# yahoojapan/srgd

Hardware: AMD Instinct MI355X
Metric: HR tiles/sec (256->1024 x4, 50 steps, CFG=1.0) (higher is better)
Workload: dtype bf16; 1 GPU; BASELINE configs[1]: one 256x256 LR tile x4 SR per step, 50 DDPM steps, class_cond_scale=1.0, dim-128 U-Net, bf16, device Philox noise; 5 steps (HR tiles) advance in lock-step so their U-Net tiles share launches; images_in_lockstep=5, step_lanes=1, tiles_per_unet_launch=125, parallelism=image-sharded x1

## Files before the change

srgd_amd/csrc/conv1x1_bf16.hip:

```cpp
#include "conv1x1_epilogue.hpp"

namespace srgd {
namespace {

constexpr int BM1 = 256, BN1 = 128, KC1 = 32, NT1 = 512;
constexpr int A1_BYTES = BM1 * KC1 * 2;
constexpr int B1_BYTES = BN1 * KC1 * 2;
constexpr int STAGE1 = A1_BYTES + B1_BYTES;
constexpr int RING1 = 3;
constexpr int LDS1_BYTES = RING1 * STAGE1;
static_assert(LDS1_BYTES >= EPI_LDS_BYTES && BM1 == EPI_BM && BN1 == EPI_BN && NT1 == EPI_NT, "conv1x1_epilogue.hpp tile shape");

typedef __attribute__((address_space(3))) void* lds_ptr1;
__device__ __forceinline__ void dma16_1(__amdgpu_buffer_rsrc_t rsrc, char* lds_wave_base, int voffset, int soffset) {
  __builtin_amdgcn_raw_ptr_buffer_load_lds(rsrc, (lds_ptr1)lds_wave_base, 16, voffset, soffset, 0, 0);
}
#define WAIT_VM1(N) asm volatile("s_waitcnt vmcnt(" #N ")" ::: "memory")
#define BARRIER1()                       \
  do {                                   \
    __builtin_amdgcn_s_barrier();        \
    __builtin_amdgcn_sched_barrier(0);   \
  } while (0)

struct Conv1Args {
  const bf16* in0; const bf16* in1; int C0, C1;
  int B, Hin, Win;
  int Hout, Wout;
  int KH, KW, stride;
  int ps0, ps1;
  const bf16* w;
  const float* bias;
  int Cout;
  bf16* out;
  const bf16* aux;
  const float* gn_a; const float* gn_b;
  unsigned char* oq; unsigned char* os;
  float* eps4; const float* fin_w; const float* fin_b;
};

__device__ __forceinline__ int row_swz1(int row) { return (row >> 1) & 3; }

template <int EPI>
__global__ __launch_bounds__(NT1, 4) void conv1x1_bf16_kernel(Conv1Args p) {
  extern __shared__ __attribute__((aligned(16))) char smem[];
  const int tid = threadIdx.x;
  const int lane = tid & 63;
  const int wave = __builtin_amdgcn_readfirstlane(tid >> 6);
  const int wm = wave >> 1, wn = wave & 1;
  const int r16 = lane & 15, q16 = lane >> 4;

  const int n_tiles = p.Cout / BN1;
  const int HWo = p.Hout * p.Wout;
  int wg = blockIdx.x;
  {
    const int nwg = gridDim.x, q = nwg >> 3, rem = nwg & 7, x = wg & 7, k = wg >> 3;
    wg = (x < rem ? x * (q + 1) : rem * (q + 1) + (x - rem) * q) + k;
  }
  const int nt = wg % n_tiles;
  const int mt = wg / n_tiles;
  const long m0 = (long)mt * BM1;
  const int b = (int)(m0 / HWo);
  const int p0 = (int)(m0 - (long)b * HWo);
  const int Cin = p.C0 + p.C1;
  const int CC = Cin / KC1;
  const int S = p.KH * p.KW * CC;

#define K_A1_DECL(J)                                                      \
  int a_b0##J, a_b1##J;                                                      \
  {                                                                          \
    const int g = (wave + 8 * J) * 64 + lane;                                \
    const int P = g >> 2;                                                    \
    const int op = p0 + P;                                                   \
    const int oy = op / p.Wout, ox = op - oy * p.Wout;                       \
    const int pix = oy * p.stride * p.Win + ox * p.stride;                   \
    const int sub = (g & 3) ^ row_swz1(P);                                   \
    a_b0##J = (pix * p.ps0 + sub * 8) * 2;                                   \
    a_b1##J = (pix * p.ps1 + sub * 8) * 2;                                   \
  }
  K_A1_DECL(0) K_A1_DECL(1)
#undef K_A1_DECL
  const size_t img0 = (size_t)p.Hin * p.Win * p.ps0, img1 = (size_t)p.Hin * p.Win * p.ps1;
  const __amdgpu_buffer_rsrc_t rs0 =
      __builtin_amdgcn_make_buffer_rsrc((void*)(p.in0 + (size_t)b * img0), 0, (int)(img0 * 2), 0x00020000);
  const __amdgpu_buffer_rsrc_t rs1 = __builtin_amdgcn_make_buffer_rsrc(
      (void*)(p.in1 ? p.in1 + (size_t)b * img1 : p.in0), 0, p.in1 ? (int)(img1 * 2) : 0, 0x00020000);
  const size_t w_tile_stride = (size_t)n_tiles * B1_BYTES;
  const __amdgpu_buffer_rsrc_t rsw = __builtin_amdgcn_make_buffer_rsrc(
      (void*)((const char*)p.w + (size_t)nt * B1_BYTES), 0, (int)((size_t)(S - 1) * w_tile_stride + B1_BYTES), 0x00020000);

  int i_ty = 0, i_tx = 0, i_cc = 0, i_slot = 0, i_w = 0;
  const int tid16 = tid * 16;
  auto issue = [&]() __attribute__((always_inline)) {
    const int c = i_cc * KC1;
    const bool first = c < p.C0;
    const int soff = first ? ((i_ty * p.Win + i_tx) * p.ps0 + c) * 2 : ((i_ty * p.Win + i_tx) * p.ps1 + c - p.C0) * 2;
    char* st = smem + i_slot * STAGE1;
    const int vo0 = first ? a_b00 : a_b10, vo1 = first ? a_b01 : a_b11;
    if (first) {
      dma16_1(rs0, st + wave * 1024, vo0, soff);
      dma16_1(rs0, st + (wave + 8) * 1024, vo1, soff);
    } else {
      dma16_1(rs1, st + wave * 1024, vo0, soff);
      dma16_1(rs1, st + (wave + 8) * 1024, vo1, soff);
    }
    dma16_1(rsw, st + A1_BYTES + wave * 1024, tid16, i_w);
    i_w += (int)w_tile_stride;
    i_slot = i_slot == RING1 - 1 ? 0 : i_slot + 1;
    if (++i_cc == CC) {
      i_cc = 0;
      if (++i_tx == p.KW) { i_tx = 0; ++i_ty; }
    }
  };

  f32x4 c00 = 0, c01 = 0, c02 = 0, c03 = 0, c10 = 0, c11 = 0, c12 = 0, c13 = 0,
        c20 = 0, c21 = 0, c22 = 0, c23 = 0, c30 = 0, c31 = 0, c32 = 0, c33 = 0;
  auto a_addr = [&](int i) {
    const int P = wm * 64 + i * 16 + r16;
    return P * 64 + ((q16 ^ row_swz1(P)) << 4);
  };
  auto b_addr = [&](int j) {
    const int n = wn * 64 + j * 16 + r16;
    return A1_BYTES + n * 64 + ((q16 ^ row_swz1(n)) << 4);
  };
  const int aa0 = a_addr(0), aa1 = a_addr(1), aa2 = a_addr(2), aa3 = a_addr(3);
  const int ba0 = b_addr(0), ba1 = b_addr(1), ba2 = b_addr(2), ba3 = b_addr(3);
  int c_slot = 0;
  auto compute = [&]() __attribute__((always_inline)) {
    const char* st = smem + c_slot * STAGE1;
    c_slot = c_slot == RING1 - 1 ? 0 : c_slot + 1;
    const bf16x8 a0 = *reinterpret_cast<const bf16x8*>(st + aa0);
    const bf16x8 a1 = *reinterpret_cast<const bf16x8*>(st + aa1);
    const bf16x8 a2 = *reinterpret_cast<const bf16x8*>(st + aa2);
    const bf16x8 a3 = *reinterpret_cast<const bf16x8*>(st + aa3);
    const bf16x8 b0 = *reinterpret_cast<const bf16x8*>(st + ba0);
    const bf16x8 b1 = *reinterpret_cast<const bf16x8*>(st + ba1);
    const bf16x8 b2 = *reinterpret_cast<const bf16x8*>(st + ba2);
    const bf16x8 b3 = *reinterpret_cast<const bf16x8*>(st + ba3);
#define MM(C_, A_, B_) C_ = __builtin_amdgcn_mfma_f32_16x16x32_bf16(A_, B_, C_, 0, 0, 0)
    MM(c00, a0, b0); MM(c01, a0, b1); MM(c02, a0, b2); MM(c03, a0, b3);
    MM(c10, a1, b0); MM(c11, a1, b1); MM(c12, a1, b2); MM(c13, a1, b3);
    MM(c20, a2, b0); MM(c21, a2, b1); MM(c22, a2, b2); MM(c23, a2, b3);
    MM(c30, a3, b0); MM(c31, a3, b1); MM(c32, a3, b2); MM(c33, a3, b3);
#undef MM
  };

  issue();
  if (S > 1) issue();
  if (S > 1) WAIT_VM1(3); else WAIT_VM1(0);
  BARRIER1();
  for (int s = 0; s < S; ++s) {
    if (s + 2 < S) issue();
    compute();
    if (s + 2 < S) WAIT_VM1(3); else WAIT_VM1(0);
    BARRIER1();
  }

  conv1x1_epilogue<EPI, BM1>(p, smem, tid, nt, m0, b, p0, c00, c01, c02, c03, c10, c11, c12, c13, c20, c21, c22, c23, c30, c31, c32, c33);
}

}

bool conv1x1_bf16_eligible(const ConvArgs& a) {
  if (a.pad != 0 || a.stride < 1 || a.KH < 1 || a.KW < 1) return false;
  if ((a.Hout - 1) * a.stride + a.KH > a.Hin || (a.Wout - 1) * a.stride + a.KW > a.Win) return false;
  if (a.ps0 % 8 || (a.C1 && (a.ps1 % 8 || a.ps1 < a.C1))) return false;
  if (a.ps0 != a.C0 && (a.C1 || (long)(a.Win - (a.Wout - 1) * a.stride - a.KW) * a.ps0 + a.ps0 < a.C0)) return false;
  if (a.C1 && (a.KH != 1 || a.KW != 1)) return false;
  if (a.C0 % KC1 || a.C1 % KC1 || a.Cout % BN1 || a.Cout != a.CoutPad) return false;
  if (((long)a.Hout * a.Wout) % BM1) return false;
  if (a.gn_partial) return false;
  if (a.mode == CONV_PIXEL_SHUFFLE_SILU && ((a.Cout / 4) % BN1 || a.residual || a.gn_res_src)) return false;
  if (a.mode != CONV_PLAIN && a.mode != CONV_PIXEL_SHUFFLE_SILU) return false;
  if (a.residual && a.gn_res_src) return false;
  if (a.eps4 && (!a.gn_res_src || a.Cout != BN1 || !a.fin_w || !a.fin_b || a.out_q)) return false;
  if ((size_t)a.Hin * a.Win * (size_t)std::max(a.ps0, a.ps1) * 2 >= (1ull << 31)) return false;
  if ((size_t)a.KH * a.KW * ((a.C0 + a.C1) / KC1) * (a.Cout / BN1) * B1_BYTES >= (1ull << 31)) return false;
  return true;
}

void pack_conv1x1_bf16(const float* src_tap_o_i, int taps, int Cin, int Cout, std::vector<unsigned short>& out,
                       unsigned short (*to_bf16)(float)) {
  const int CC = Cin / KC1, NTL = Cout / BN1;
  out.assign((size_t)taps * CC * NTL * BN1 * KC1, 0);
  for (int tap = 0; tap < taps; ++tap)
    for (int cc = 0; cc < CC; ++cc)
      for (int nt = 0; nt < NTL; ++nt) {
        unsigned short* tile = out.data() + ((size_t)(tap * CC + cc) * NTL + nt) * BN1 * KC1;
        for (int n = 0; n < BN1; ++n)
          for (int c = 0; c < 4; ++c) {
            const int cs = c ^ ((n >> 1) & 3);
            for (int e = 0; e < 8; ++e) {
              const int ci = cc * KC1 + c * 8 + e, o = nt * BN1 + n;
              tile[n * KC1 + cs * 8 + e] = to_bf16(src_tap_o_i[((size_t)tap * Cout + o) * Cin + ci]);
            }
          }
      }
}

int conv1x1_bf16(const ConvArgs& a, const void* packed_w, hipStream_t st) {
  if (!conv1x1_bf16_eligible(a)) SRGD_FAIL("conv1x1_bf16: shape not eligible");
  Conv1Args p;
  p.in0 = (const bf16*)a.in0; p.in1 = (const bf16*)a.in1; p.C0 = a.C0; p.C1 = a.C1;
  p.B = a.B; p.Hin = a.Hin; p.Win = a.Win; p.Hout = a.Hout; p.Wout = a.Wout;
  p.KH = a.KH; p.KW = a.KW; p.stride = a.stride; p.ps0 = a.ps0; p.ps1 = a.C1 ? a.ps1 : 0;
  p.w = (const bf16*)packed_w; p.bias = a.bias; p.Cout = a.Cout; p.out = (bf16*)a.out;
  p.aux = a.gn_res_src ? (const bf16*)a.gn_res_src : (const bf16*)a.residual;
  p.gn_a = a.gn_res_a; p.gn_b = a.gn_res_b;
  p.oq = (unsigned char*)a.out_q; p.os = (unsigned char*)a.out_s;
  p.eps4 = a.eps4; p.fin_w = a.fin_w; p.fin_b = a.fin_b;
  if ((p.oq != nullptr) != (p.os != nullptr)) SRGD_FAIL("conv1x1_bf16: MX-fp8 twin needs both the element and the scale buffer");
  const long m_tiles = (long)a.B * a.Hout * a.Wout / BM1;
  const long grid = m_tiles * (a.Cout / BN1);
  if (grid <= 0 || grid > 0x7fffffffL) SRGD_FAIL("conv1x1_bf16: bad grid");
  static bool attr_set[64] = {};
  if (DeviceSetup once(attr_set); once.need) {
#define K_SET1(E_)                                                                                   \
  SRGD_HIP(hipFuncSetAttribute(reinterpret_cast<const void*>(&conv1x1_bf16_kernel<E_>),                 \
                               hipFuncAttributeMaxDynamicSharedMemorySize, LDS1_BYTES));
    K_SET1(EPI_PLAIN) K_SET1(EPI_RESIDUAL) K_SET1(EPI_GNTAIL) K_SET1(EPI_PS_SILU) K_SET1(EPI_GNTAIL_FINAL)
#undef K_SET1
    once.done();
  }
#define K_GO1(E_) hipLaunchKernelGGL((conv1x1_bf16_kernel<E_>), dim3((unsigned)grid), dim3(NT1), LDS1_BYTES, st, p)
  if (a.mode == CONV_PIXEL_SHUFFLE_SILU) K_GO1(EPI_PS_SILU);
  else if (a.gn_res_src && a.eps4) K_GO1(EPI_GNTAIL_FINAL);
  else if (a.gn_res_src) K_GO1(EPI_GNTAIL);
  else if (a.residual) K_GO1(EPI_RESIDUAL);
  else K_GO1(EPI_PLAIN);
#undef K_GO1
  SRGD_HIP(hipGetLastError());
  return 0;
}

}
```

Before: 1.357 HR tiles/s.

## Make conv1x1 kernel persistent with wave-private epilogue overlapping next tile loads

Turns the 1x1/strided conv GEMM kernel into a persistent kernel whose grid is capped at resident workgroups, each looping over output tiles. The prefetch of the next tile's K-steps continues through the epilogue, and the epilogue now uses per-wave private LDS staging instead of the shared ring, so stores of one tile overlap loads of the next. This is meant to remove the per-tile launch and tail costs and the pipeline drain at each tile boundary. In exchange it adds LDS per workgroup, which could lower occupancy, and it adds hand-tuned vmcnt bookkeeping. The final GN-tail variant keeps the old one-tile path.

```diff
diff --git a/srgd_amd/csrc/conv1x1_bf16.hip b/srgd_amd/csrc/conv1x1_bf16.hip
--- a/srgd_amd/csrc/conv1x1_bf16.hip
+++ b/srgd_amd/csrc/conv1x1_bf16.hip
@@ -1,4 +1,4 @@
-#include "conv1x1_epilogue.hpp"
+#include "conv1x1_epilogue_wave.hpp"
 
 namespace srgd {
 namespace {
@@ -8,8 +8,10 @@
 constexpr int B1_BYTES = BN1 * KC1 * 2;
 constexpr int STAGE1 = A1_BYTES + B1_BYTES;
 constexpr int RING1 = 3;
-constexpr int LDS1_BYTES = RING1 * STAGE1;
-static_assert(LDS1_BYTES >= EPI_LDS_BYTES && BM1 == EPI_BM && BN1 == EPI_BN && NT1 == EPI_NT, "conv1x1_epilogue.hpp tile shape");
+constexpr int RING1_BYTES = RING1 * STAGE1;
+constexpr int LDS1_BYTES = RING1_BYTES + (NT1 / 64) * WEPI_STG_BYTES;
+static_assert(RING1_BYTES >= EPI_LDS_BYTES && BM1 == EPI_BM && BN1 == EPI_BN && NT1 == EPI_NT, "conv1x1_epilogue.hpp tile shape");
+static_assert(2 * LDS1_BYTES <= 160 * 1024, "two workgroups per CU");
 
 typedef __attribute__((address_space(3))) void* lds_ptr1;
 __device__ __forceinline__ void dma16_1(__amdgpu_buffer_rsrc_t rsrc, char* lds_wave_base, int voffset, int soffset) {
@@ -31,6 +33,7 @@
   const bf16* w;
   const float* bias;
   int Cout;
+  int n_wg_tiles;
   bf16* out;
   const bf16* aux;
   const float* gn_a; const float* gn_b;
@@ -51,46 +54,55 @@
 
   const int n_tiles = p.Cout / BN1;
   const int HWo = p.Hout * p.Wout;
-  int wg = blockIdx.x;
-  {
-    const int nwg = gridDim.x, q = nwg >> 3, rem = nwg & 7, x = wg & 7, k = wg >> 3;
-    wg = (x < rem ? x * (q + 1) : rem * (q + 1) + (x - rem) * q) + k;
-  }
-  const int nt = wg % n_tiles;
-  const int mt = wg / n_tiles;
-  const long m0 = (long)mt * BM1;
-  const int b = (int)(m0 / HWo);
-  const int p0 = (int)(m0 - (long)b * HWo);
   const int Cin = p.C0 + p.C1;
   const int CC = Cin / KC1;
   const int S = p.KH * p.KW * CC;
-
-#define K_A1_DECL(J)                                                      \
-  int a_b0##J, a_b1##J;                                                      \
+  const int T = p.n_wg_tiles;
+  auto tile_of = [&](int v, int& nt_, int& b_, int& p0_) {
+    const int q = T >> 3, rem = T & 7, x = v & 7, k = v >> 3;
+    const int wg = (x < rem ? x * (q + 1) : rem * (q + 1) + (x - rem) * q) + k;
+    nt_ = wg % n_tiles;
+    const int mt = wg / n_tiles, tpi = HWo / BM1;
+    b_ = mt / tpi;
+    p0_ = (mt - b_ * tpi) * BM1;
+  };
+
+  const size_t img0 = (size_t)p.Hin * p.Win * p.ps0, img1 = (size_t)p.Hin * p.Win * p.ps1;
+  const size_t w_tile_stride = (size_t)n_tiles * B1_BYTES;
+  int i_v = blockIdx.x, i_ty = 0, i_tx = 0, i_cc = 0, i_slot = 0, i_w = 0;
+  int a_b00 = 0, a_b10 = 0, a_b01 = 0, a_b11 = 0;
+  __amdgpu_buffer_rsrc_t rs0, rs1, rsw;
+  auto issue_tile = [&]() __attribute__((always_inline)) {
+    int nt_, b_, p0_;
+    tile_of(i_v, nt_, b_, p0_);
+    unsigned zero = 0;
+    unsigned wout = (unsigned)p.Wout;
+    asm volatile("" : "+v"(zero), "+s"(wout));
+    const int ln = (int)__builtin_amdgcn_mbcnt_hi(~0u, __builtin_amdgcn_mbcnt_lo(~0u, zero));
+#define K_A1_SET(J)                                                          \
   {                                                                          \
-    const int g = (wave + 8 * J) * 64 + lane;                                \
+    const int g = (wave + 8 * J) * 64 + ln;                                  \
     const int P = g >> 2;                                                    \
-    const int op = p0 + P;                                                   \
-    const int oy = op / p.Wout, ox = op - oy * p.Wout;                       \
-    const int pix = oy * p.stride * p.Win + ox * p.stride;                   \
+    const unsigned op = (unsigned)(p0_ + P);                                 \
+    const unsigned oy = op / wout, ox = op - oy * wout;                      \
+    const int pix = (int)oy * p.stride * p.Win + (int)ox * p.stride;         \
     const int sub = (g & 3) ^ row_swz1(P);                                   \
     a_b0##J = (pix * p.ps0 + sub * 8) * 2;                                   \
     a_b1##J = (pix * p.ps1 + sub * 8) * 2;                                   \
   }
-  K_A1_DECL(0) K_A1_DECL(1)
-#undef K_A1_DECL
-  const size_t img0 = (size_t)p.Hin * p.Win * p.ps0, img1 = (size_t)p.Hin * p.Win * p.ps1;
-  const __amdgpu_buffer_rsrc_t rs0 =
-      __builtin_amdgcn_make_buffer_rsrc((void*)(p.in0 + (size_t)b * img0), 0, (int)(img0 * 2), 0x00020000);
-  const __amdgpu_buffer_rsrc_t rs1 = __builtin_amdgcn_make_buffer_rsrc(
-      (void*)(p.in1 ? p.in1 + (size_t)b * img1 : p.in0), 0, p.in1 ? (int)(img1 * 2) : 0, 0x00020000);
-  const size_t w_tile_stride = (size_t)n_tiles * B1_BYTES;
-  const __amdgpu_buffer_rsrc_t rsw = __builtin_amdgcn_make_buffer_rsrc(
-      (void*)((const char*)p.w + (size_t)nt * B1_BYTES), 0, (int)((size_t)(S - 1) * w_tile_stride + B1_BYTES), 0x00020000);
-
-  int i_ty = 0, i_tx = 0, i_cc = 0, i_slot = 0, i_w = 0;
+    K_A1_SET(0) K_A1_SET(1)
+#undef K_A1_SET
+    rs0 = __builtin_amdgcn_make_buffer_rsrc((void*)(p.in0 + (size_t)b_ * img0), 0, (int)(img0 * 2), 0x00020000);
+    rs1 = __builtin_amdgcn_make_buffer_rsrc((void*)(p.in1 ? p.in1 + (size_t)b_ * img1 : p.in0), 0, p.in1 ? (int)(img1 * 2) : 0, 0x00020000);
+    rsw = __builtin_amdgcn_make_buffer_rsrc((void*)((const char*)p.w + (size_t)nt_ * B1_BYTES), 0,
+                                            (int)((size_t)(S - 1) * w_tile_stride + B1_BYTES), 0x00020000);
+    i_ty = i_tx = i_cc = 0;
+    i_w = 0;
+  };
+  issue_tile();
   const int tid16 = tid * 16;
-  auto issue = [&]() __attribute__((always_inline)) {
+  auto issue = [&]() __attribute__((always_inline)) -> bool {
+    if (i_v >= T) return false;
     const int c = i_cc * KC1;
     const bool first = c < p.C0;
     const int soff = first ? ((i_ty * p.Win + i_tx) * p.ps0 + c) * 2 : ((i_ty * p.Win + i_tx) * p.ps1 + c - p.C0) * 2;
@@ -108,12 +120,18 @@
     i_slot = i_slot == RING1 - 1 ? 0 : i_slot + 1;
     if (++i_cc == CC) {
       i_cc = 0;
-      if (++i_tx == p.KW) { i_tx = 0; ++i_ty; }
-    }
-  };
-
-  f32x4 c00 = 0, c01 = 0, c02 = 0, c03 = 0, c10 = 0, c11 = 0, c12 = 0, c13 = 0,
-        c20 = 0, c21 = 0, c22 = 0, c23 = 0, c30 = 0, c31 = 0, c32 = 0, c33 = 0;
+      if (++i_tx == p.KW) {
+        i_tx = 0;
+        if (++i_ty == p.KH) {
+          i_v = EPI == EPI_GNTAIL_FINAL ? T : i_v + (int)gridDim.x;
+          if (i_v < T) issue_tile();
+        }
+      }
+    }
+    return true;
+  };
+
+  f32x4 c00, c01, c02, c03, c10, c11, c12, c13, c20, c21, c22, c23, c30, c31, c32, c33;
   auto a_addr = [&](int i) {
     const int P = wm * 64 + i * 16 + r16;
     return P * 64 + ((q16 ^ row_swz1(P)) << 4);
@@ -144,18 +162,34 @@
 #undef MM
   };
 
-  issue();
-  if (S > 1) issue();
-  if (S > 1) WAIT_VM1(3); else WAIT_VM1(0);
+  bool more = issue();
+  more = issue() && more;
+  if (more) WAIT_VM1(3); else WAIT_VM1(0);
   BARRIER1();
-  for (int s = 0; s < S; ++s) {
-    if (s + 2 < S) issue();
-    compute();
-    if (s + 2 < S) WAIT_VM1(3); else WAIT_VM1(0);
-    BARRIER1();
-  }
-
-  conv1x1_epilogue<EPI, BM1>(p, smem, tid, nt, m0, b, p0, c00, c01, c02, c03, c10, c11, c12, c13, c20, c21, c22, c23, c30, c31, c32, c33);
+  for (int v = blockIdx.x; v < T; v += gridDim.x) {
+    int nt, b, p0;
+    tile_of(v, nt, b, p0);
+    c00 = 0; c01 = 0; c02 = 0; c03 = 0; c10 = 0; c11 = 0; c12 = 0; c13 = 0;
+    c20 = 0; c21 = 0; c22 = 0; c23 = 0; c30 = 0; c31 = 0; c32 = 0; c33 = 0;
+    for (int s = 0; s < S; ++s) {
+      const bool issued = issue();
+      compute();
+      if (!issued) WAIT_VM1(0);
+      else if (s == 0 && v != (int)blockIdx.x) WAIT_VM1(11);
+      else WAIT_VM1(3);
+      BARRIER1();
+    }
+    static_assert(WEPI_STORES + 3 == 11, "vmcnt of a later tile's first K-step");
+
+    if constexpr (EPI == EPI_GNTAIL_FINAL) {
+      conv1x1_epilogue<EPI, BM1>(p, smem, tid, nt, (long)b * HWo + p0, b, p0, c00, c01, c02, c03, c10, c11, c12, c13, c20, c21, c22, c23,
+                                 c30, c31, c32, c33);
+      break;
+    } else {
+      conv1x1_epilogue_wave<EPI>(p, smem + RING1_BYTES + wave * WEPI_STG_BYTES, wm, wn, nt, b, p0, c00, c01, c02, c03, c10, c11, c12, c13,
+                                 c20, c21, c22, c23, c30, c31, c32, c33);
+    }
+  }
 }
 
 }
@@ -210,22 +244,41 @@
   p.eps4 = a.eps4; p.fin_w = a.fin_w; p.fin_b = a.fin_b;
   if ((p.oq != nullptr) != (p.os != nullptr)) SRGD_FAIL("conv1x1_bf16: MX-fp8 twin needs both the element and the scale buffer");
   const long m_tiles = (long)a.B * a.Hout * a.Wout / BM1;
-  const long grid = m_tiles * (a.Cout / BN1);
-  if (grid <= 0 || grid > 0x7fffffffL) SRGD_FAIL("conv1x1_bf16: bad grid");
+  const long tiles = m_tiles * (a.Cout / BN1);
+  if (tiles <= 0 || tiles > 0x7fffffffL) SRGD_FAIL("conv1x1_bf16: bad grid");
+  p.n_wg_tiles = (int)tiles;
+  const int epi = a.mode == CONV_PIXEL_SHUFFLE_SILU ? EPI_PS_SILU
+                : a.gn_res_src ? (a.eps4 ? EPI_GNTAIL_FINAL : EPI_GNTAIL)
+                : a.residual ? EPI_RESIDUAL : EPI_PLAIN;
   static bool attr_set[64] = {};
+  static int slots[64][5] = {};
+  int dev = 0;
+  SRGD_HIP(hipGetDevice(&dev));
+  if (dev < 0 || dev >= 64) SRGD_FAIL("conv1x1_bf16: device index out of range");
   if (DeviceSetup once(attr_set); once.need) {
-#define K_SET1(E_)                                                                                   \
-  SRGD_HIP(hipFuncSetAttribute(reinterpret_cast<const void*>(&conv1x1_bf16_kernel<E_>),                 \
-                               hipFuncAttributeMaxDynamicSharedMemorySize, LDS1_BYTES));
+    int n_cu = 0;
+    SRGD_HIP(hipDeviceGetAttribute(&n_cu, hipDeviceAttributeMultiprocessorCount, dev));
+#define K_SET1(E_)                                                                                                          \
+  {                                                                                                                         \
+    const void* fn = reinterpret_cast<const void*>(&conv1x1_bf16_kernel<E_>);                                               \
+    SRGD_HIP(hipFuncSetAttribute(fn, hipFuncAttributeMaxDynamicSharedMemorySize, LDS1_BYTES));                              \
+    int per_cu = 0;                                                                                                         \
+    SRGD_HIP(hipOccupancyMaxActiveBlocksPerMultiprocessor(&per_cu, fn, NT1, LDS1_BYTES));                                   \
+    if (per_cu < 1 || n_cu < 1) SRGD_FAIL("conv1x1_bf16: the kernel does not fit on a CU");                                 \
+    const long n = (long)per_cu * n_cu;                                                                                     \
+    __atomic_store_n(&slots[dev][E_], (int)(n > 8 ? n & ~7L : 8), __ATOMIC_RELAXED);                                        \
+  }
     K_SET1(EPI_PLAIN) K_SET1(EPI_RESIDUAL) K_SET1(EPI_GNTAIL) K_SET1(EPI_PS_SILU) K_SET1(EPI_GNTAIL_FINAL)
 #undef K_SET1
     once.done();
   }
+  const long resident = __atomic_load_n(&slots[dev][epi], __ATOMIC_RELAXED);
+  const long grid = (epi == EPI_GNTAIL_FINAL || tiles <= resident) ? tiles : resident;
 #define K_GO1(E_) hipLaunchKernelGGL((conv1x1_bf16_kernel<E_>), dim3((unsigned)grid), dim3(NT1), LDS1_BYTES, st, p)
-  if (a.mode == CONV_PIXEL_SHUFFLE_SILU) K_GO1(EPI_PS_SILU);
-  else if (a.gn_res_src && a.eps4) K_GO1(EPI_GNTAIL_FINAL);
-  else if (a.gn_res_src) K_GO1(EPI_GNTAIL);
-  else if (a.residual) K_GO1(EPI_RESIDUAL);
+  if (epi == EPI_PS_SILU) K_GO1(EPI_PS_SILU);
+  else if (epi == EPI_GNTAIL_FINAL) K_GO1(EPI_GNTAIL_FINAL);
+  else if (epi == EPI_GNTAIL) K_GO1(EPI_GNTAIL);
+  else if (epi == EPI_RESIDUAL) K_GO1(EPI_RESIDUAL);
   else K_GO1(EPI_PLAIN);
 #undef K_GO1
   SRGD_HIP(hipGetLastError());
diff --git a/srgd_amd/csrc/conv1x1_epilogue_wave.hpp b/srgd_amd/csrc/conv1x1_epilogue_wave.hpp
--- /dev/null
+++ b/srgd_amd/csrc/conv1x1_epilogue_wave.hpp
@@ -0,0 +1,125 @@
+#pragma once
+#include "conv1x1_epilogue.hpp"
+
+namespace srgd {
+namespace {
+
+constexpr int WEPI_STG_BYTES = 1024;
+constexpr int WEPI_STORES = 8;
+
+template <int EPI, class Args>
+__device__ __forceinline__ void conv1x1_epilogue_wave(const Args& p, char* stg, const int wm, const int wn, const int nt,
+                                                      const int b, const int p0,
+                                                      const f32x4& c00, const f32x4& c01, const f32x4& c02, const f32x4& c03,
+                                                      const f32x4& c10, const f32x4& c11, const f32x4& c12, const f32x4& c13,
+                                                      const f32x4& c20, const f32x4& c21, const f32x4& c22, const f32x4& c23,
+                                                      const f32x4& c30, const f32x4& c31, const f32x4& c32, const f32x4& c33) {
+  static_assert(EPI == EPI_PLAIN || EPI == EPI_RESIDUAL || EPI == EPI_GNTAIL || EPI == EPI_PS_SILU, "wave-private epilogue variants");
+  unsigned zero = 0;
+  unsigned wout = (unsigned)p.Wout;
+  asm volatile("" : "+v"(zero), "+s"(wout));
+  const int lane = (int)__builtin_amdgcn_mbcnt_hi(~0u, __builtin_amdgcn_mbcnt_lo(~0u, zero));
+  const int r16 = lane & 15, q16 = lane >> 4;
+  const int row8 = lane >> 3, c8 = lane & 7;
+  const int ch0 = nt * EPI_BN + wn * 64 + c8 * 8;
+  const int pl0 = p0 + wm * 64 + row8;
+  const size_t o0 = ((size_t)b * p.Hout * p.Wout + pl0) * p.Cout + ch0;
+  const size_t rstep = (size_t)8 * p.Cout;
+
+  float bias[4] = {0.f, 0.f, 0.f, 0.f};
+  if (p.bias) {
+#pragma unroll
+    for (int ni = 0; ni < 4; ++ni) bias[ni] = p.bias[nt * EPI_BN + wn * 64 + ni * 16 + r16];
+  }
+  bf16x8 auxv[8];
+  f32x4 a_lo = {0.f, 0.f, 0.f, 0.f}, a_hi = a_lo, b_lo = a_lo, b_hi = a_lo;
+  if (EPI == EPI_RESIDUAL || EPI == EPI_GNTAIL) {
+#pragma unroll
+    for (int r = 0; r < 4; ++r) auxv[r] = __builtin_nontemporal_load(reinterpret_cast<const bf16x8*>(p.aux + o0 + r * rstep));
+  }
+
+  const bool odd_lane = (r16 & 1) != 0;
+  unsigned w0[4][4], w1[4][4];
+#pragma unroll
+  for (int ni = 0; ni < 4; ++ni) {
+    const float bs = bias[ni];
+#pragma unroll
+    for (int mi = 0; mi < 4; ++mi) {
+      const f32x4 av = mi == 0 ? (ni == 0 ? c00 : ni == 1 ? c01 : ni == 2 ? c02 : c03)
+                     : mi == 1 ? (ni == 0 ? c10 : ni == 1 ? c11 : ni == 2 ? c12 : c13)
+                     : mi == 2 ? (ni == 0 ? c20 : ni == 1 ? c21 : ni == 2 ? c22 : c23)
+                               : (ni == 0 ? c30 : ni == 1 ? c31 : ni == 2 ? c32 : c33);
+      float v0 = av[0] + bs, v1 = av[1] + bs, v2 = av[2] + bs, v3 = av[3] + bs;
+      if (EPI == EPI_PS_SILU) { v0 = silu<false>(v0); v1 = silu<false>(v1); v2 = silu<false>(v2); v3 = silu<false>(v3); }
+      typedef __bf16 bf16x2_t __attribute__((ext_vector_type(2)));
+      const unsigned own01 = __builtin_bit_cast(unsigned, __builtin_convertvector(f32x2{v0, v1}, bf16x2_t));
+      const unsigned own23 = __builtin_bit_cast(unsigned, __builtin_convertvector(f32x2{v2, v3}, bf16x2_t));
+      const unsigned recv = (unsigned)__builtin_amdgcn_update_dpp(0, (int)(odd_lane ? own01 : own23), 0xB1, 0xf, 0xf, true);
+      const unsigned lo_ch = odd_lane ? recv : own01, hi_ch = odd_lane ? own23 : recv;
+      w0[mi][ni] = __builtin_amdgcn_perm(hi_ch, lo_ch, 0x05040100u);
+      w1[mi][ni] = __builtin_amdgcn_perm(hi_ch, lo_ch, 0x07060302u);
+    }
+  }
+
+  if (EPI == EPI_RESIDUAL || EPI == EPI_GNTAIL) {
+    __builtin_amdgcn_sched_barrier(0);
+    if (EPI == EPI_GNTAIL) {
+      const float* ga = p.gn_a + (size_t)b * p.Cout + ch0;
+      const float* gb = p.gn_b + (size_t)b * p.Cout + ch0;
+      a_lo = *reinterpret_cast<const f32x4*>(ga); a_hi = *reinterpret_cast<const f32x4*>(ga + 4);
+      b_lo = *reinterpret_cast<const f32x4*>(gb); b_hi = *reinterpret_cast<const f32x4*>(gb + 4);
+    }
+#pragma unroll
+    for (int r = 4; r < 8; ++r) auxv[r] = __builtin_nontemporal_load(reinterpret_cast<const bf16x8*>(p.aux + o0 + r * rstep));
+  }
+
+  const int wk = (q16 & 1) * 2 + (odd_lane ? 1 : 0);
+  char* const wbase = stg + wk * 256 + ((r16 >> 3) << 4) + (((r16 >> 1) & 3) << 2);
+  const char* const rbase = stg + row8 * 128 + ((c8 ^ (((row8 >> 1) & 3) << 1)) << 4);
+  int CoutPS = 0, ps_ij = 0, ps_c0 = 0;
+  if (EPI == EPI_PS_SILU) {
+    CoutPS = p.Cout >> 2;
+    ps_ij = (nt * EPI_BN) / CoutPS;
+    ps_c0 = nt * EPI_BN - ps_ij * CoutPS + wn * 64 + c8 * 8;
+  }
+#pragma unroll
+  for (int r = 0; r < 8; ++r) {
+    const int mi = r >> 1, h = r & 1;
+    if ((q16 >> 1) == h) {
+#pragma unroll
+      for (int ni = 0; ni < 4; ++ni) {
+        char* const a = wbase + ((ni ^ wk) << 5);
+        *reinterpret_cast<unsigned*>(a) = w0[mi][ni];
+        *reinterpret_cast<unsigned*>(a + 128) = w1[mi][ni];
+      }
+    }
+    asm volatile("" ::: "memory");
+    bf16x8 v = *reinterpret_cast<const bf16x8*>(rbase);
+    asm volatile("" ::: "memory");
+    size_t o;
+    if (EPI == EPI_PS_SILU) {
+      const unsigned op = (unsigned)(pl0 + 8 * r);
+      const unsigned oy = op / wout, ox = op - oy * wout;
+      o = ((size_t)(b * 2 * p.Hout + 2 * (int)oy + (ps_ij >> 1)) * (2 * p.Wout) + 2 * ox + (ps_ij & 1)) * CoutPS + ps_c0;
+    } else {
+      o = o0 + r * rstep;
+      if (EPI == EPI_RESIDUAL) {
+        const bf16x8 rr = auxv[r];
+#pragma unroll
+        for (int e = 0; e < 8; ++e) v[e] = (bf16)((float)v[e] + (float)rr[e]);
+      } else if (EPI == EPI_GNTAIL) {
+        const bf16x8 hh = auxv[r];
+#pragma unroll
+        for (int e = 0; e < 8; ++e) {
+          const float ca = e < 4 ? a_lo[e & 3] : a_hi[e & 3], cb = e < 4 ? b_lo[e & 3] : b_hi[e & 3];
+          v[e] = (bf16)(silu<false>(ca * (float)hh[e] + cb) + (float)v[e]);
+        }
+      }
+    }
+    __builtin_nontemporal_store(v, reinterpret_cast<bf16x8*>(p.out + o));
+    if (p.oq) mx_store_twin(v, p.oq, p.os, o, lane & 3);
+  }
+}
+
+}
+}
```

Result: no change. 1.356 HR tiles/s (-0.1%).
